# xuanvinh1997/llm-fp8

Measured on AMD Instinct MI355X. Metric: train tokens/sec + FP8 GEMM % of MFMA peak, Llama-3.2-3B seq512 b16, higher is better.
Workload: dtype fp8 (E4M3/E5M2 operands, fp32 accumulate, bf16 activations); 1 GPU; llama-3.2-3b (28 layers) full fine-tuning step, batch 16/GPU x seq 512, fp8_scenario=default (te_llama counterpart, lm_head FP8 under the outer recipe), random-init weights, synthetic tokens; route=fused, global_batch=16, seq_len=512, parallelism=single

## Files before the change

include/mi_fp8.h:

```cpp
#ifndef MI_FP8_H
#define MI_FP8_H

#include <stdint.h>

#ifdef __cplusplus
extern "C" {
#endif

#define MI_FMT_E4M3 0
#define MI_FMT_E5M2 1

#define MI_OK 0
#define MI_ERR_ARG (-1)
#define MI_ERR_SHAPE (-2)
#define MI_ERR_HIP (-3)

#define MI_OUT_BF16 0
#define MI_OUT_F32 1

#define MI_AMAX_ALGO_MAX 0
#define MI_AMAX_ALGO_MOST_RECENT 1

#define MI_ABI_VERSION 5
#define MI_ABI_REVISION 4
int mi_abi_version(void);
int mi_abi_revision(void);
const char* mi_last_error(void);
int mi_device_supported(void);

int mi_cast_amax(const void* x_bf16, void* y_fp8, void* yT_fp8, const float* scale, float* amax,
                 int64_t rows, int64_t cols, int64_t ld_y, int64_t ld_yT, int fmt, void* stream);
int mi_transpose_u8(const void* y, void* yT, int64_t rows, int64_t cols, int64_t ld_y, int64_t ld_yT, void* stream);
int mi_cast_amax_colsum(const void* x_bf16, void* y_fp8, void* yT_fp8, const float* scale, float* amax,
                        float* colsum_partial, int64_t rows, int64_t cols, int64_t ld_y, int64_t ld_yT, int fmt, void* stream);
int mi_colsum_finish(const float* partial, int64_t P, int64_t C, void* out, int out_dtype, void* stream);
int mi_colsum_finish_multi(const void* const* partials, const int64_t* P, const int64_t* C, void* const* outs,
                           const int* out_dtypes, int n, void* stream);

int mi_scale_update(float* amax_history, float* scale, float* scale_inv, const float* fp8_max,
// ... 119 lines not shown
                       const float* grad_scale, float lr, float beta1, float beta2, float eps, float weight_decay,
                       int64_t step, int sink_kind, void* stream);

int mi_adamw_sr_bf16_multi(const int64_t* table, int n_tensors, const int32_t* chunks, int n_chunks, int chunk_elems,
                           const float* grad_scale, float lr, float beta1, float beta2, float eps, float weight_decay,
                           int64_t step, int sink_kind, uint64_t seed, void* stream);

int mi_embedding_grad_add(void* grad_bf16, const void* dy_bf16, const int64_t* sorted_ids, const int64_t* perm, int64_t tokens,
                          int64_t hidden, int64_t vocab, float alpha, int64_t padding_idx, void* stream);
int mi_adamw_bf16(void* p_bf16, const void* g_bf16, void* exp_avg_bf16, void* exp_avg_sq_bf16, int64_t n,
                  const float* grad_scale, float lr, float beta1, float beta2, float eps, float weight_decay,
                  int64_t step, void* stream);

int mi_attn_fwd(const void* q, const void* k, const void* v, void* o, float* lse, int B, int S, int H, int G, int D,
                int64_t q_ts, int64_t k_ts, int64_t v_ts, int64_t o_ts, float scale, int causal, void* stream);
typedef struct mi_gemm_plan {
  int algo, family, build, sched, mx, tile_cfg, tiles_m, tiles_n, grid_x, grid_y, block, one_tile_per_wg, sk_units, bias_use;
} mi_gemm_plan;
#ifdef MI_DIAG
int mi_attn_fwd_diag(const void* q, const void* k, const void* v, void* o, float* lse, unsigned long long* dbg, int B, int S,
                     int H, int G, int D, int64_t q_ts, int64_t k_ts, int64_t v_ts, int64_t o_ts, float scale, void* stream);
int mi_gemm_plan_diag(int entry, int64_t M, int64_t N, int64_t K, int64_t lda, int64_t ldb, int64_t ldd, int fmt_a, int fmt_b,
                      int out_dtype, int has_bias, int algo, mi_gemm_plan* out);
#endif
int mi_attn_bwd(const void* q, const void* k, const void* v, const void* o, const void* dout, const float* lse,
                float* delta, void* dq, void* dk, void* dv, int B, int S, int H, int G, int D, int64_t q_ts,
                int64_t k_ts, int64_t v_ts, int64_t o_ts, int64_t do_ts, int64_t dq_ts, int64_t dk_ts, int64_t dv_ts,
                float scale, int causal, void* stream);

#ifdef __cplusplus
// ... 4 lines not shown
```

llm_fp8_amd/_lib.py:

```python
from __future__ import annotations

import ctypes
import os

_HERE = os.path.dirname(os.path.abspath(__file__))
LIB_PATH = os.environ.get("LLM_FP8_AMD_LIB") or os.path.join(_HERE, "libmi_fp8.so")
LAB_LIB_PATH = os.path.join(os.path.dirname(_HERE), "tools", "bin", "libmi_fp8_lab.so")

MI_FMT_E4M3 = 0
MI_FMT_E5M2 = 1
ABI_VERSION = 5
ABI_REVISION = 4

_c_i64 = ctypes.c_int64
_c_int = ctypes.c_int
_p = ctypes.c_void_p

class GemmProblem(ctypes.Structure):
    _fields_ = [("A", ctypes.c_void_p), ("B", ctypes.c_void_p), ("D", ctypes.c_void_p), ("sa_inv", ctypes.c_void_p),
                ("sb_inv", ctypes.c_void_p), ("M", ctypes.c_int64), ("N", ctypes.c_int64), ("K", ctypes.c_int64),
                ("lda", ctypes.c_int64), ("ldb", ctypes.c_int64), ("ldd", ctypes.c_int64)]


class GemmMxProblem(ctypes.Structure):
    _fields_ = [("A", ctypes.c_void_p), ("SA", ctypes.c_void_p), ("B", ctypes.c_void_p), ("SB", ctypes.c_void_p),
                ("D", ctypes.c_void_p), ("M", ctypes.c_int64), ("N", ctypes.c_int64), ("K", ctypes.c_int64)]

# ... 58 lines not shown
REVISION_SIGNATURES = {
    "mi_abi_revision": [],
    "mi_adamw_f32_multi": [_p, _c_int, _p, _c_int, _c_int, _p, ctypes.c_float, ctypes.c_float, ctypes.c_float, ctypes.c_float,
                           ctypes.c_float, _c_i64, _c_int, _p],
    "mi_amax_bf16": [_p, _p, _c_int, _c_i64, _c_i64, _p],
    "mi_amax_norm": [_p, _p, _p, _p, _c_int, _c_i64, _c_i64, _p],
    "mi_amax_swiglu": [_p, _p, _p, _c_int, _c_i64, _c_i64, _p],
    "mi_amax_dswiglu": [_p, _p, _p, _p, _c_int, _c_i64, _c_i64, _p],
    "mi_current_scale": [_p, _c_int, ctypes.c_float, ctypes.c_float, _c_int, _p, _p],
    "mi_blockfp8_quantize_ex": [_p, _p, _p, _p, _p, _p, _c_i64, _c_i64, _c_i64, _c_int, _c_int, ctypes.c_float, _p],
    "mi_blockfp8_norm_quantize": [_p, _p, _p, _p, _p, _p, _p, _c_i64, _c_i64, _c_int, _c_int, ctypes.c_float, _p],
    "mi_blockfp8_swiglu_quantize": [_p, _p, _p, _p, _p, _c_i64, _c_i64, _c_int, _c_int, ctypes.c_float, _p],
    "mi_blockfp8_dswiglu_quantize": [_p, _p, _p, _p, _p, _p, _p, _c_i64, _c_i64, _c_int, _c_int, ctypes.c_float, _p],
    "mi_adamw_sr_bf16_multi": [_p, _c_int, _p, _c_int, _c_int, _p, ctypes.c_float, ctypes.c_float, ctypes.c_float, ctypes.c_float,
                               ctypes.c_float, _c_i64, _c_int, ctypes.c_uint64, _p],
}
SIGNATURES.update(REVISION_SIGNATURES)
LAB_SIGNATURES = {
    "mi_attn_fwd_diag": [_p, _p, _p, _p, _p, _p, _c_int, _c_int, _c_int, _c_int, _c_int, _c_i64, _c_i64, _c_i64, _c_i64, ctypes.c_float, _p],
    "mi_gemm_plan_diag": [_c_int] + [_c_i64] * 6 + [_c_int] * 5 + [ctypes.POINTER(GemmPlan)],
}

_lib = None


def _bind(path: str, signatures) -> ctypes.CDLL:
    lib = ctypes.CDLL(path)
    for name, argtypes in signatures.items():
        if name in REVISION_SIGNATURES and not hasattr(lib, name):
            continue
# ... 54 lines not shown
```

llm_fp8_amd/csrc/mi_attn.hip:

```cpp
#include "mi_common.h"

namespace mi {

typedef __bf16 bf8 __attribute__((ext_vector_type(8)));
typedef short s4v __attribute__((ext_vector_type(4)));
typedef short s8v __attribute__((ext_vector_type(8)));
typedef float f16v __attribute__((ext_vector_type(16)));
typedef __attribute__((address_space(3))) s4v lds_s4v;

template <int D>
__device__ __forceinline__ int tile_off(int row, int ch) {
  if (D == 128) return 256 * row + 16 * (ch ^ (((row & 3) << 2) | ((row >> 2) & 3)));
  return 128 * row + 16 * (ch ^ (((row & 1) << 2) | ((row >> 1) & 3)));
}

__device__ __forceinline__ bf8 as_bf8(v4i v) { return __builtin_bit_cast(bf8, v); }

template <int D>
__device__ __forceinline__ bf8 row_frag(const char* tile, int r0, int t, int lane) {
  const int r = lane & 31, h = lane >> 5;
  return as_bf8(*reinterpret_cast<const v4i*>(tile + tile_off<D>(r0 + r, 2 * t + h)));
}

template <int D>
// ... 47 lines not shown
    __builtin_amdgcn_raw_ptr_buffer_load_lds(rs, MI_LDS_PTR(tile + (4 * i + w) * 1024), 16, voff[i], soff, 0, 0);
}
template <int D>
__device__ __forceinline__ void stage_dma_checked(rsrc_t rs, const int* voff, int adv, char* tile, int w) {
#pragma unroll
  for (int i = 0; i < D / 32; ++i)
    __builtin_amdgcn_raw_ptr_buffer_load_lds(rs, MI_LDS_PTR(tile + (4 * i + w) * 1024), 16, (int)((u32)voff[i] + (u32)adv), 0, 0, 0);
}
template <int D, bool TAIL>
__device__ __forceinline__ void stage_tile(rsrc_t rs, const int* voff, int adv, char* tile, int w) {
  if (TAIL) stage_dma_checked<D>(rs, voff, adv, tile, w);
  else stage_dma<D>(rs, voff, adv, tile, w);
}
__device__ __forceinline__ void dma_wait_all() { asm volatile("s_waitcnt vmcnt(0)" ::: "memory"); }

template <int D, bool CAUSAL, bool DIAG = false, bool TAIL = false>
__global__ __launch_bounds__(256, 2) void attn_fwd_kernel(const uint16_t* __restrict__ q, const uint16_t* __restrict__ k,
                                                          const uint16_t* __restrict__ v, uint16_t* __restrict__ o,
                                                          float* __restrict__ lse, int S, int H, int G, int64_t q_ts,
                                                          int64_t k_ts, int64_t v_ts, int64_t o_ts, float c,
                                                          unsigned long long* __restrict__ dbg = nullptr) {
  constexpr int TILE = ATT_KB * D * 2;
  constexpr int KT = D / 16, DB = D / 32;
  __shared__ __attribute__((aligned(16))) char lds[4 * TILE];
  const int tid = threadIdx.x, lane = tid & 63, w = tid >> 6, r = lane & 31, h = lane >> 5;
  const int qb = gridDim.x - 1 - blockIdx.x, head = blockIdx.y, b = blockIdx.z, g = head / (H / G);
  const int q_first = qb * ATT_QB + w * 32;
  const int qrow = q_first + r;
  int ntiles = CAUSAL ? (qb * ATT_QB + ATT_QB) / ATT_KB : S / ATT_KB;
  if (TAIL) {
    const int stiles = (S + ATT_KB - 1) / ATT_KB;
    ntiles = CAUSAL ? min(ntiles, stiles) : stiles;
  }
  const uint16_t* kbase = k + (int64_t)b * S * k_ts + (int64_t)g * D;
  const uint16_t* vbase = v + (int64_t)b * S * v_ts + (int64_t)g * D;

// ... 126 lines not shown
    MI_STAMP(2)
    dma_wait_all();
    MI_STAMP(3)
    __syncthreads();
    MI_STAMP(4)
  }
  if (DIAG && dbg != nullptr && lane == 0) {
    unsigned long long* dp = dbg + ((((int64_t)b * H + head) * gridDim.x + qb) * 4 + w) * 8;
    for (int i2 = 0; i2 < 5; ++i2) dp[i2] = tsum[i2];
    dp[5] = (unsigned long long)ntiles;
  }
#undef MI_STAMP

  l += __shfl_xor(l, 32);
  const float inv = 1.0f / l;
  if (h == 0 && (!TAIL || qrow < S)) lse[((int64_t)b * H + head) * S + qrow] = m * c + __builtin_amdgcn_logf(l);
  char* ot = lds + w * (32 * D * 2);
#pragma unroll
  for (int d = 0; d < DB; ++d)
#pragma unroll
    for (int i = 0; i < 4; ++i) {
      const int ch = 4 * d + i;
      uint2 pk;
      pk.x = pack_bf16x2(oacc[d][4 * i] * inv, oacc[d][4 * i + 1] * inv);
      pk.y = pack_bf16x2(oacc[d][4 * i + 2] * inv, oacc[d][4 * i + 3] * inv);
      *reinterpret_cast<uint2*>(ot + r * (D * 2) + 16 * (ch ^ (r & (D / 8 - 1))) + 8 * h) = pk;
    }
  __builtin_amdgcn_s_waitcnt(0xc07f);
  __builtin_amdgcn_wave_barrier();
  constexpr int CPR = D / 8;
#pragma unroll
  for (int it = 0; it < 32 * CPR / 64; ++it) {
    const int idx = it * 64 + lane, row = idx / CPR, ch = idx % CPR;
    const v4i val = *reinterpret_cast<const v4i*>(ot + row * (D * 2) + 16 * (ch ^ (row & (CPR - 1))));
    if (!TAIL || q_first + row < S) *reinterpret_cast<v4i*>(o + ((int64_t)b * S + q_first + row) * o_ts + (int64_t)head * D + ch * 8) = val;
  }
}


template <int D, bool TAIL = false>
__device__ __forceinline__ void store_rows_from_accT(const f16v (&acc)[D / 32], float mul, char* slice, uint16_t* out,
                                                     int64_t row_stride, int lane, int nrows = 32) {
  const int r = lane & 31, h = lane >> 5;
  constexpr int CPR = D / 8;
#pragma unroll
  for (int d = 0; d < D / 32; ++d)
#pragma unroll
    for (int i = 0; i < 4; ++i) {
      const int ch = 4 * d + i;
      uint2 pk;
// ... 304 lines not shown
#define MI_ATTN_FWD_T(DD, CC, TT)                                                                                      \
  hipLaunchKernelGGL((mi::attn_fwd_kernel<DD, CC, false, TT>), grid, block, 0, st, (const uint16_t*)q, (const uint16_t*)k, \
                     (const uint16_t*)v, (uint16_t*)o, lse, S, H, G, q_ts, k_ts, v_ts, o_ts, c, (unsigned long long*)nullptr)
#define MI_ATTN_FWD(DD, CC)                                                                                            \
  do {                                                                                                                 \
    if (tail) MI_ATTN_FWD_T(DD, CC, true); else MI_ATTN_FWD_T(DD, CC, false);                                          \
  } while (0)
  if (D == 128) {
    if (causal) MI_ATTN_FWD(128, true); else MI_ATTN_FWD(128, false);
  } else {
    if (causal) MI_ATTN_FWD(64, true); else MI_ATTN_FWD(64, false);
  }
#undef MI_ATTN_FWD_T
#undef MI_ATTN_FWD
  MI_CHECK_LAUNCH("mi_attn_fwd launch");
  return MI_OK;
}

#ifdef MI_DIAG
extern "C" int mi_attn_fwd_diag(const void* q, const void* k, const void* v, void* o, float* lse, unsigned long long* dbg, int B,
                                int S, int H, int G, int D, int64_t q_ts, int64_t k_ts, int64_t v_ts, int64_t o_ts, float scale,
                                void* stream) {
  MI_CHECK_ARG(q && k && v && o && lse && dbg, "mi_attn_fwd_diag: null pointer");
  MI_CHECK_ARG(D == 128 && S % 128 == 0 && H % G == 0, "mi_attn_fwd_diag: unsupported shape");
  dim3 grid(S / mi::ATT_QB, H, B), block(256);
  hipLaunchKernelGGL((mi::attn_fwd_kernel<128, true, true>), grid, block, 0, (hipStream_t)stream, (const uint16_t*)q,
                     (const uint16_t*)k, (const uint16_t*)v, (uint16_t*)o, lse, S, H, G, q_ts, k_ts, v_ts, o_ts,
                     scale * 1.4426950408889634f, dbg);
  MI_CHECK_LAUNCH("mi_attn_fwd_diag launch");
  return MI_OK;
// ... 46 lines not shown
```

llm_fp8_amd/pytorch/attention.py:

```python
from __future__ import annotations

import os
import weakref
from typing import Optional

import torch
import torch.nn.functional as F

from . import ops
from .module import DyHandoff, LayerNormLinear, Linear, handoff_readers

__all__ = ["RotaryPositionEmbedding", "apply_rotary_pos_emb", "DotProductAttention", "MultiheadAttention"]


class RotaryPositionEmbedding(torch.nn.Module):

    def __init__(self, dim: int, rotary_percent: float = 1.0, seq_len_interpolation_factor=None,
                 pretrained_max_position_embeddings=None, rotary_base: float = 10000.0):
        super().__init__()
        if rotary_percent < 1.0:
            dim = int(dim * rotary_percent)
        self.dim = dim
        self.seq_len_interpolation_factor = seq_len_interpolation_factor
        inv_freq = 1.0 / (rotary_base ** (torch.arange(0, dim, 2, dtype=torch.float32) / dim))
# ... 68 lines not shown
            if h.mx:
                fp8 = ops.mxfp8_rope_bwd_quantize(*args, h.fmt, rowwise=h.want_y, colwise=h.want_t)
            else:
                fp8 = ops.rope_qkv_backward_cast(*args, h.scale, h.amax, h.fmt, want_y=h.want_y, want_t=h.want_t)
            g = torch.empty((B, S, (n_q + 2 * n_kv) * d), dtype=torch.bfloat16, device=dq.device)
            h.put(fp8, g)
            return g, None, None, None, None, None, None
        g = ops.rope_qkv_backward(dq.reshape(T, n_q * d), dk.reshape(T, n_kv * d), dv.reshape(T, n_kv * d), cos, sin,
                                  n_q, n_kv, d, S)
        return g.view(B, S, -1), None, None, None, None, None, None


class _FlashAttnFn(torch.autograd.Function):

    @staticmethod
    def forward(ctx, q, k, v, scale, causal):
        o, lse = ops.attn_fwd(q, k, v, scale, causal)
        ctx.save_for_backward(q, k, v, o, lse)
        ctx.scale, ctx.causal = scale, causal
        return o

    @staticmethod
    def backward(ctx, do):
        q, k, v, o, lse = ctx.saved_tensors
        ok = (do.stride(3) == 1 and do.stride(2) == do.shape[3] and do.stride(0) == do.shape[1] * do.stride(1)
              and do.stride(1) % 8 == 0 and do.data_ptr() % 16 == 0)
        do = do if ok else do.clone(memory_format=torch.contiguous_format)
        dq, dk, dv = ops.attn_bwd(do, q, k, v, o, lse, ctx.scale, ctx.causal)
        return dq, dk, dv, None, None


def _flash_ok(q, k, v, causal: bool, dropout: float) -> bool:
    if not (q.is_cuda and q.dtype == k.dtype == v.dtype == torch.bfloat16 and dropout == 0.0 and causal):
        return False
    B, S, H, D = q.shape
    if D not in (64, 128) or S % 16 or S < 128 or H % k.shape[2]:
        return False
    return all(t.stride(3) == 1 and t.stride(2) == D and t.stride(0) == S * t.stride(1) and t.stride(1) % 8 == 0
               and S * t.stride(1) * 2 < 2 ** 31 and t.data_ptr() % 16 == 0 for t in (q, k, v))


class DotProductAttention(torch.nn.Module):

    def __init__(self, num_attention_heads: int, kv_channels: int, num_gqa_groups: Optional[int] = None,
                 attention_dropout: float = 0.0, attn_mask_type: str = "causal", qkv_format: str = "bshd", **_ignored):
        super().__init__()
        self.h, self.d = num_attention_heads, kv_channels
        self.g = num_gqa_groups or num_attention_heads
        self.p, self.attn_mask_type, self.qkv_format = attention_dropout, attn_mask_type, qkv_format

    def forward(self, q, k, v, attention_mask=None):
        if self.qkv_format == "sbhd":
            q, k, v = (t.transpose(0, 1) for t in (q, k, v))
        causal = self.attn_mask_type in ("causal", "padding_causal")
        if _flash_ok(q, k, v, causal, self.p if self.training else 0.0):
            o = _FlashAttnFn.apply(q, k, v, self.d ** -0.5, True)
            if self.qkv_format == "sbhd":
                o = o.transpose(0, 1)
            return o.reshape(*o.shape[:2], self.h * self.d)
        q, k, v = (t.transpose(1, 2) for t in (q, k, v))
        mask = None
        if not causal and attention_mask is not None:
            mask = ~attention_mask if attention_mask.dtype == torch.bool else attention_mask
        o = F.scaled_dot_product_attention(q, k, v, attn_mask=mask, dropout_p=self.p if self.training else 0.0,
                                           is_causal=causal, enable_gqa=(self.g != self.h))
        o = o.transpose(1, 2)
        if self.qkv_format == "sbhd":
            o = o.transpose(0, 1)
        return o.reshape(*o.shape[:2], self.h * self.d)


# ... 37 lines not shown
            if not self.input_layernorm:
                return self._attend(self.qkv(hidden_states), attention_mask, rotary_pos_emb), hidden_states
            handoff = DyHandoff() if (rotary_pos_emb is not None and hidden_states.is_cuda and torch.is_grad_enabled()
                                      and os.environ.get("LLM_FP8_AMD_NO_DY_HANDOFF") != "1") else None
            qkv, skip = self.layernorm_qkv(hidden_states, _with_skip=True, _rstd=_rstd, _dy_handoff=handoff)
            return self._attend(qkv, attention_mask, rotary_pos_emb, handoff), skip
        qkv = self.layernorm_qkv(hidden_states) if self.input_layernorm else self.qkv(hidden_states)
        return self._attend(qkv, attention_mask, rotary_pos_emb)

    def _attend(self, qkv: torch.Tensor, attention_mask, rotary_pos_emb, handoff=None) -> torch.Tensor:
        if (rotary_pos_emb is not None and not isinstance(rotary_pos_emb, (tuple, list)) and qkv.is_cuda
                and qkv.dtype == torch.bfloat16 and self.qkv_format == "bshd" and self.d % 16 == 0
                and rotary_pos_emb.shape[-1] == self.d):
            cos, sin = _cos_sin_tables(rotary_pos_emb, qkv.shape[1])
            q, k, v = _RoPESplitFn.apply(qkv, cos, sin, self.h, self.g, self.d, handoff)
            return self.proj(self.core_attention(q, k, v, attention_mask))
        if handoff is not None:
            handoff.withdraw()
        q, k, v = torch.split(qkv, self.split, dim=-1)
        a, b = qkv.shape[0], qkv.shape[1]
        q = q.reshape(a, b, self.h, self.d)
        k = k.reshape(a, b, self.g, self.d)
        v = v.reshape(a, b, self.g, self.d)
        if rotary_pos_emb is not None:
            fq, fk = rotary_pos_emb if isinstance(rotary_pos_emb, (tuple, list)) else (rotary_pos_emb, rotary_pos_emb)
            q = apply_rotary_pos_emb(q, fq, self.qkv_format)
            k = apply_rotary_pos_emb(k, fk, self.qkv_format)
        ctx = self.core_attention(q, k, v, attention_mask)
        return self.proj(ctx)
```

llm_fp8_amd/pytorch/module.py:

```python
from __future__ import annotations

import io
import os
from typing import List, Optional, Sequence, Tuple

import torch
import torch.nn.functional as F

from ..common.recipe import DelayedScaling, Float8BlockScaling, Float8CurrentScaling, Format, MXFP8BlockScaling, Recipe, fmt_codes
from . import ops
from .fp8 import FP8GlobalStateManager, ModuleMeta

__all__ = ["Linear", "LayerNormLinear", "LayerNormMLP", "LayerNorm", "RMSNorm"]


def _as_bf16_2d(t: torch.Tensor) -> torch.Tensor:
    t2 = t.reshape(-1, t.shape[-1])
    if t2.dtype != torch.bfloat16:
        t2 = t2.to(torch.bfloat16)
    return t2.contiguous()


class DyHandoff:
    __slots__ = ("scale", "amax", "fmt", "want_y", "want_t", "fp8", "ptr", "mx", "act_ref")
# ... 11 lines not shown

    def offered(self) -> bool:
        return (self.scale is not None or self.mx) and (self.want_y or self.want_t)

    def put(self, fp8: tuple, placeholder: torch.Tensor):
        self.fp8, self.ptr = fp8, placeholder.untyped_storage().data_ptr()

    def take(self, dy: torch.Tensor):
        if dy.untyped_storage().data_ptr() != self.ptr:
            raise RuntimeError("DyHandoff: the gradient reaching the Linear is not the producer's placeholder "
                               "(an op was inserted between the q|k|v projection and the rotary split)")
        fp8, self.fp8, self.ptr = self.fp8, None, None
        return fp8


def handoff_readers(t) -> bool:
    if torch.is_anomaly_enabled():
        return True
    if t is None:
        return False
    return bool(getattr(t, "retains_grad", False)) or bool(getattr(t, "_backward_hooks", None))


class _GemmSpec:
    __slots__ = ("recipe", "meta_fwd", "meta_bwd", "g", "fmt_fwd", "fmt_bwd", "trigger_bwd_update", "training", "eps",
                 "wcache", "first_mb", "with_skip", "rstd", "dy_handoff", "defer_bias", "q")

    def __init__(self, recipe, meta_fwd, meta_bwd, g, trigger_bwd_update, training, eps=1e-5, wcache=None, first_mb=None,
                 with_skip=False, rstd=None, dy_handoff=None, defer_bias=False):
        self.dy_handoff = dy_handoff
        self.defer_bias = defer_bias
        self.eps = eps
        self.rstd = rstd
        self.with_skip = with_skip
        self.wcache, self.first_mb = wcache, first_mb
        self.recipe, self.meta_fwd, self.meta_bwd, self.g = recipe, meta_fwd, meta_bwd, g
        self.fmt_fwd, self.fmt_bwd = fmt_codes(recipe.fp8_format)
        if recipe.mxfp8():
            self.q = _MXQ(self.fmt_fwd, self.fmt_bwd)
        elif recipe.current():
            self.q = _CurrentQ(recipe, self.fmt_fwd, self.fmt_bwd)
        elif recipe.block():
            self.q = _BlockQ(recipe, self.fmt_fwd, self.fmt_bwd)
        else:
            self.q = _DelayedQ(meta_fwd, meta_bwd, self.fmt_fwd, self.fmt_bwd)
# ... 101 lines not shown
    swiglu_adds_bias = True
    colsum_dtypes = None

    def __init__(self, mf, mb, fmt_f: int, fmt_b: int):
        self.mf, self.mb, self.fmt_f, self.fmt_b = mf, mb, fmt_f, fmt_b

    def _act(self, y, yT, s: int):
        return (y, self.mf.scale_inv(s)), (yT, self.mf.scale_inv_snapshot()[s:s + 1])

    def quantize(self, x2, g: int, want_t: bool, norm=None):
        mf, s = self.mf, 3 * g
        if norm is None:
            return self._act(*ops.cast_amax(x2, mf.scale(s), mf.amax(s), self.fmt_f, want_t=want_t), s)
        return self._act(*ops.norm_cast(x2, norm[0], norm[1], mf.scale(s), mf.amax(s), self.fmt_f, want_t=want_t), s)

    def swiglu(self, h, g: int, want_t: bool, bias):
        mf, s = self.mf, 3 * g
        return self._act(*ops.swiglu_cast(h, mf.scale(s), mf.amax(s), self.fmt_f, want_t=want_t, bias=bias), s)

    def _grad(self, y, yT, cs, s: int):
        si = self.mb.scale_inv(s)
        return (y, si), (yT, si), cs

    def quantize_grad(self, g2, g: int, want_y: bool, want_t: bool, colsum: bool = False):
        mb, s = self.mb, 2 * g
        out = ops.cast_amax(g2, mb.scale(s), mb.amax(s), self.fmt_b, want_y=want_y, want_t=want_t, want_colsum=colsum)
        return self._grad(out[0], out[1], out[2] if colsum else None, s)

    def dswiglu(self, h, dact, g: int, want_y: bool, want_t: bool, colsum: bool, bias):
        mb, s = self.mb, 2 * g
# ... 64 lines not shown

    def quantize_grad(self, g2, g: int, want_y: bool, want_t: bool, colsum: bool = False):
        q = ops.mxfp8_quantize(g2, self.fmt_b, rowwise=want_y, colwise=want_t, want_colsum=colsum)
        return q[:2], q[2:4], q[4] if colsum else None

    def dswiglu(self, h, dact, g: int, want_y: bool, want_t: bool, colsum: bool, bias):
        assert bias is None
        q = ops.mxfp8_dswiglu_quantize(h, dact, self.fmt_b, rowwise=want_y, colwise=want_t, want_colsum=colsum)
        return q[:2], q[2:4], q[4]

    def offer(self, handoff: DyHandoff, g: int, want_y: bool, want_t: bool) -> None:
        handoff.offer(None, None, self.fmt_b, want_y, want_t, mx=True)

    def taken(self, fp8, g: int):
        return fp8[:2], fp8[2:], None

    def operands(self, a, b):
        return a + b

    def gemm(self, a, b, bias):
        return ops.gemm_mxfp8(a[0], a[1], b[0], b[1], self.fmt_f, self.fmt_f, bias=bias)

    def unflat(self, flat):
        return flat[:2], flat[2:]

    def quantize_weights(self, weights, ns, N: int, K: int, dev, g: int, want_t: bool):
        fmt = self.fmt_f
        ws_ = [(w if w.dtype == torch.bfloat16 else w.to(torch.bfloat16)).contiguous() for w in weights]
        if len(ws_) == 1:
            return ops.mxfp8_quantize(ws_[0], fmt, rowwise=True, colwise=want_t)
# ... 135 lines not shown
        return (out[0], t3[2:3]), (out[1], t3[2:3]), out[2] if colsum else None

    def dswiglu(self, h, dact, g: int, want_y: bool, want_t: bool, colsum: bool, bias):
        part = ops.amax_partial(h.device, ops.amax_grid(h.shape[0], h.shape[1] // 2, 32))
        ops.amax_dswiglu(h, bias, dact, part)
        t3 = self._triple(part, self.fmt_b, self.recipe.fp8_quant_bwd_grad)
        y, yT, cs = ops.dswiglu_cast(h, dact, t3[1:2], None, self.fmt_b, want_y=want_y, want_t=want_t, want_colsum=colsum, bias=bias)
        return (y, t3[2:3]), (yT, t3[2:3]), cs

    def offer(self, handoff: DyHandoff, g: int, want_y: bool, want_t: bool) -> None:
        """Nothing: a DyHandoff producer needs the scale of grad_output before it has produced it.  RoPE backward and cross-entropy
        backward take their bf16 route and the Linear quantises the gradient it receives."""

    def taken(self, fp8, g: int):
        raise RuntimeError("Float8CurrentScaling offers no DyHandoff, so no producer can have put FP8 copies into one")

    operands = _DelayedQ.operands
    gemm = _DelayedQ.gemm
    unflat = _DelayedQ.unflat

    def quantize_weights(self, weights, ns, N: int, K: int, dev, g: int, want_t: bool):
        ws_ = [(w if w.dtype == torch.bfloat16 else w.to(torch.bfloat16)).contiguous() for w in weights]
        grids = [ops.amax_grid(n, K) for n in ns]
        part = ops.amax_partial(dev, sum(grids))
        o = 0
        for w, n in zip(ws_, grids):
            ops.amax_bf16(w, part[o:o + n])
            o += n
        t3 = self._triple(part, self.fmt_f, self.recipe.fp8_quant_fwd_weight)
        w8 = torch.empty((N, K), dtype=torch.uint8, device=dev)
# ... 108 lines not shown
    dx = gemm(*dgrad, fmt_b, fmt_f) if need_dgrad else None
    dw = gemm(*wgrad, fmt_b, fmt_f, out=dw_out) if need_wgrad else None
    return dx, dw


def _skip_2d(dskip: Optional[torch.Tensor], like: torch.Tensor) -> Optional[torch.Tensor]:
    if dskip is None:
        return None
    d = dskip.reshape(like.shape)
    return d if (d.dtype == torch.bfloat16 and d.is_contiguous()) else d.to(torch.bfloat16).contiguous()


def _quantize_input(ctx, spec: _GemmSpec, x2, ln_w, want_t: bool, need_dgrad: bool):
    ctx.norm = None
    if ln_w is None:
        return spec.q.quantize(x2, spec.g, want_t)
    gam = (ln_w if ln_w.dtype == torch.bfloat16 else ln_w.to(torch.bfloat16)).contiguous()
    rstd = spec.rstd if spec.rstd is not None else ops.rmsnorm_stats(x2, spec.eps)
    if need_dgrad:
        ctx.norm = (x2, rstd, gam, ln_w.dtype)
    return spec.q.quantize(x2, spec.g, want_t, (rstd, gam))


def _finish_dx(ctx, dx, dskip, colsums=None):
    dln = None
    if ctx.norm is not None and dx is not None:
        xin, rstd, gam, ln_dtype = ctx.norm
        ctx.norm = None
        dx, dln = ops.rmsnorm_bwd(dx, xin, rstd, gam, dres=_skip_2d(dskip, dx), dgamma_dtype=ln_dtype, finish=colsums is None)
        dskip = None
# ... 231 lines not shown
        torch.nn.init.normal_(w, mean=0.0, std=0.023)
    return torch.nn.Parameter(w)


class Linear(_FP8Module):

    def __init__(self, in_features: int, out_features: int, bias: bool = True, params_dtype=None, device="cuda",
                 init_method=None, **_ignored):
        super().__init__()
        self.in_features, self.out_features = in_features, out_features
        dt = params_dtype or torch.get_default_dtype()
        self.weight = _init_weight((out_features, in_features), dt, device, init_method)
        self.bias = torch.nn.Parameter(torch.zeros(out_features, dtype=dt, device=device)) if bias else None
        self.use_bias = bias

    def forward(self, inp: torch.Tensor, is_first_microbatch=None) -> torch.Tensor:
        st = self._prepare(inp.device)
        if st is None:
            if getattr(self, "_pending_norm", None) is not None:
                raise RuntimeError("Linear: a deferred RMSNorm is pending but FP8 is off for this forward")
            return F.linear(inp, _master(self.weight).to(inp.dtype), None if self.bias is None else self.bias.to(inp.dtype))
        handoff = DyHandoff() if (getattr(self, "offer_dy_handoff", False) and self.training and torch.is_grad_enabled()
                                  and self.bias is None) else None
        pn, self._pending_norm = getattr(self, "_pending_norm", None), None
        ln_w, eps, rstd = None, 1e-5, None
        if pn is not None:
            ln_w, eps, rs, ptr, shape = pn
            if inp.data_ptr() != ptr or tuple(inp.shape) != shape:
                raise RuntimeError("Linear: a deferred RMSNorm is pending for another tensor than the one this forward received")
            rstd = _usable_rstd(rs, inp, eps)
        y = _FP8LinearFn.apply(inp, self.bias, self._spec(st, is_first_microbatch, eps=eps, rstd=rstd, dy_handoff=handoff), ln_w,
                               self.weight)
        if handoff is not None and handoff.offered():
            y._mi_dy_handoff = handoff
        return y

    def extra_repr(self):
        return f"in_features={self.in_features}, out_features={self.out_features}, bias={self.use_bias}"


class LayerNormLinear(_FP8Module):

    def __init__(self, in_features: int, out_features: int, eps: float = 1e-5, bias: bool = True,
                 normalization: str = "LayerNorm", parameters_split=None, params_dtype=None, device="cuda",
                 zero_centered_gamma: bool = False, init_method=None, return_layernorm_output: bool = False, **_ignored):
        super().__init__()
        assert normalization in ("LayerNorm", "RMSNorm")
# ... 138 lines not shown
```

llm_fp8_amd/pytorch/ops.py:

```python
from __future__ import annotations

import ctypes
import os
from typing import Optional, Tuple

import torch

from .. import _lib
from .profiler import KernelTimer

E4M3, E5M2 = _lib.MI_FMT_E4M3, _lib.MI_FMT_E5M2
FP8_MAX = {E4M3: 448.0, E5M2: 57344.0}


_SK_WORKSPACE = {}


def ensure_gemm_workspace(device: torch.device) -> None:
    idx = device.index if device.index is not None else torch.cuda.current_device()
    if idx in _SK_WORKSPACE:
        return
    lib = _lib.load()
    with torch.cuda.device(idx):
        nbytes = int(lib.mi_gemm_workspace_bytes())
# ... 843 lines not shown
        _bshd_ok(o, D)
        assert o.shape == q.shape and lse.shape == (B, H, S) and lse.dtype == torch.float32 and lse.is_contiguous()
    args = (q.data_ptr(), k.data_ptr(), v.data_ptr(), o.data_ptr(), lse.data_ptr(), B, S, H, G, D, q.stride(1), k.stride(1),
            v.stride(1), o.stride(1), float(scale), int(causal), _stream())
    t = KernelTimer.active
    flops = 4.0 * B * H * S * S * D * (0.5 if causal else 1.0)
    if t is None:
        rc = _lib.load().mi_attn_fwd(*args)
    else:
        with t.span("attn_fwd", f"{B}x{S}x{H}x{D}", flops, 2.0 * (q.numel() * 2 + k.numel() * 2)):
            rc = _lib.load().mi_attn_fwd(*args)
    _lib.check(rc, "mi_attn_fwd")
    return o, lse


def attn_bwd(do: torch.Tensor, q: torch.Tensor, k: torch.Tensor, v: torch.Tensor, o: torch.Tensor, lse: torch.Tensor,
             scale: float, causal: bool = True, out=None):
    _dev(do, q, k, v, o, lse)
    B, S, H, D = q.shape
    G = k.shape[2]
    for t in (q, k, v, o, do):
        _bshd_ok(t, D)
    assert o.shape == do.shape == q.shape and lse.shape == (B, H, S) and lse.dtype == torch.float32 and lse.is_contiguous()
    if out is None:
        dq = torch.empty((B, S, H, D), dtype=torch.bfloat16, device=q.device)
        dk = torch.empty((B, S, G, D), dtype=torch.bfloat16, device=q.device)
        dv = torch.empty((B, S, G, D), dtype=torch.bfloat16, device=q.device)
    else:
        dq, dk, dv = out
        _dev(dq, dk, dv)
# ... 17 lines not shown
```

Baseline: 89910 tokens/s.

## Fuse FP8 cast and amax of attention output into flash-attention forward epilogue

Adds a CAST variant of the flash-attention forward kernel that, in its epilogue, converts the output tile to E4M3 with the output projection's delayed scale, publishes amax, and writes both row-major and LDS-transposed FP8 copies. A handoff object carries these copies to the o_proj Linear, which skips its own cast_amax kernel when the key matches. This removes a separate pass over the attention output and one kernel launch per layer. The cost is extra registers and LDS traffic in the attention epilogue, which could affect occupancy or scheduling, plus new Python plumbing.

```diff
diff --git a/include/mi_fp8.h b/include/mi_fp8.h
--- a/include/mi_fp8.h
+++ b/include/mi_fp8.h
@@ -22,7 +22,7 @@
 #define MI_AMAX_ALGO_MOST_RECENT 1
 
 #define MI_ABI_VERSION 5
-#define MI_ABI_REVISION 4
+#define MI_ABI_REVISION 5
 int mi_abi_version(void);
 int mi_abi_revision(void);
 const char* mi_last_error(void);
@@ -172,6 +172,9 @@
 
 int mi_attn_fwd(const void* q, const void* k, const void* v, void* o, float* lse, int B, int S, int H, int G, int D,
                 int64_t q_ts, int64_t k_ts, int64_t v_ts, int64_t o_ts, float scale, int causal, void* stream);
+int mi_attn_fwd_cast(const void* q, const void* k, const void* v, void* o, float* lse, void* y_fp8, void* yT_fp8,
+                     const float* scale_ptr, float* amax, int B, int S, int H, int G, int D, int64_t q_ts, int64_t k_ts,
+                     int64_t v_ts, int64_t ld_y, int64_t ld_yT, int fmt, float scale, int causal, void* stream);
 typedef struct mi_gemm_plan {
   int algo, family, build, sched, mx, tile_cfg, tiles_m, tiles_n, grid_x, grid_y, block, one_tile_per_wg, sk_units, bias_use;
 } mi_gemm_plan;
diff --git a/llm_fp8_amd/_lib.py b/llm_fp8_amd/_lib.py
--- a/llm_fp8_amd/_lib.py
+++ b/llm_fp8_amd/_lib.py
@@ -10,7 +10,7 @@
 MI_FMT_E4M3 = 0
 MI_FMT_E5M2 = 1
 ABI_VERSION = 5
-ABI_REVISION = 4
+ABI_REVISION = 5
 
 _c_i64 = ctypes.c_int64
 _c_int = ctypes.c_int
@@ -99,6 +99,7 @@
     "mi_blockfp8_dswiglu_quantize": [_p, _p, _p, _p, _p, _p, _p, _c_i64, _c_i64, _c_int, _c_int, ctypes.c_float, _p],
     "mi_adamw_sr_bf16_multi": [_p, _c_int, _p, _c_int, _c_int, _p, ctypes.c_float, ctypes.c_float, ctypes.c_float, ctypes.c_float,
                                ctypes.c_float, _c_i64, _c_int, ctypes.c_uint64, _p],
+    "mi_attn_fwd_cast": [_p] * 9 + [_c_int] * 5 + [_c_i64] * 5 + [_c_int, ctypes.c_float, _c_int, _p],
 }
 SIGNATURES.update(REVISION_SIGNATURES)
 LAB_SIGNATURES = {
diff --git a/llm_fp8_amd/csrc/mi_attn.hip b/llm_fp8_amd/csrc/mi_attn.hip
--- a/llm_fp8_amd/csrc/mi_attn.hip
+++ b/llm_fp8_amd/csrc/mi_attn.hip
@@ -85,12 +85,32 @@
 }
 __device__ __forceinline__ void dma_wait_all() { asm volatile("s_waitcnt vmcnt(0)" ::: "memory"); }
 
-template <int D, bool CAUSAL, bool DIAG = false, bool TAIL = false>
+struct FwdCast {
+  uint8_t* y;
+  uint8_t* yT;
+  const float* scale;
+  float* amax;
+  int64_t ld_y, ld_yT;
+};
+template <bool CAST>
+struct FwdLast { typedef unsigned long long* type; };
+template <>
+struct FwdLast<true> { typedef FwdCast type; };
+
+template <int D, bool CAUSAL, bool DIAG = false, bool TAIL = false, bool CAST = false>
 __global__ __launch_bounds__(256, 2) void attn_fwd_kernel(const uint16_t* __restrict__ q, const uint16_t* __restrict__ k,
                                                           const uint16_t* __restrict__ v, uint16_t* __restrict__ o,
                                                           float* __restrict__ lse, int S, int H, int G, int64_t q_ts,
                                                           int64_t k_ts, int64_t v_ts, int64_t o_ts, float c,
-                                                          unsigned long long* __restrict__ dbg = nullptr) {
+                                                          typename FwdLast<CAST>::type last = typename FwdLast<CAST>::type()) {
+  static_assert(!CAST || (D == 128 && CAUSAL && !DIAG && !TAIL), "the CAST form exists for head_dim 128, causal, whole blocks");
+  unsigned long long* __restrict__ dbg = nullptr;
+  if constexpr (!CAST) dbg = last;
+  float fp8_scale = 0.0f;
+  if constexpr (CAST) {
+    fp8_scale = *last.scale;
+    asm volatile("" : "+s"(fp8_scale));
+  }
   constexpr int TILE = ATT_KB * D * 2;
   constexpr int KT = D / 16, DB = D / 32;
   __shared__ __attribute__((aligned(16))) char lds[4 * TILE];
@@ -247,7 +267,7 @@
 
   l += __shfl_xor(l, 32);
   const float inv = 1.0f / l;
-  if (h == 0 && (!TAIL || qrow < S)) lse[((int64_t)b * H + head) * S + qrow] = m * c + __builtin_amdgcn_logf(l);
+  if (!CAST && h == 0 && (!TAIL || qrow < S)) lse[((int64_t)b * H + head) * S + qrow] = m * c + __builtin_amdgcn_logf(l);
   char* ot = lds + w * (32 * D * 2);
 #pragma unroll
   for (int d = 0; d < DB; ++d)
@@ -262,11 +282,71 @@
   __builtin_amdgcn_s_waitcnt(0xc07f);
   __builtin_amdgcn_wave_barrier();
   constexpr int CPR = D / 8;
+  [[maybe_unused]] u32 lo[8], hi[8];
+  [[maybe_unused]] const int rb = lane >> 4, cb = lane & 15;
+  if constexpr (CAST) {
+    v4i raw[8];
+#pragma unroll
+    for (int i = 0; i < 8; ++i) {
+      const int row = 8 * rb + i;
+      raw[i] = *reinterpret_cast<const v4i*>(ot + row * (D * 2) + 16 * (cb ^ (row & (CPR - 1))));
+    }
+    u32 screen = 0;
+#pragma unroll
+    for (int i = 0; i < 8; ++i)
+#pragma unroll
+      for (int j = 0; j < 4; ++j) screen = nan_screen(screen, (u32)raw[i][j]);
+    const bool has_nan = nan_seen(screen);
+    float amax = 0.0f;
+#pragma unroll
+    for (int i = 0; i < 8; ++i) {
+      float f[8];
+#pragma unroll
+      for (int j = 0; j < 4; ++j) {
+        const u32 wd = (u32)raw[i][j];
+        f[2 * j] = __uint_as_float(wd << 16);
+        f[2 * j + 1] = __uint_as_float(wd & 0xFFFF0000u);
+      }
+      if (__builtin_expect(has_nan, 0)) {
+#pragma unroll
+        for (int j = 0; j < 8; ++j) amax = fmaxf(amax, (f[j] != f[j]) ? 0.0f : fabsf(f[j]));
+      } else {
+#pragma unroll
+        for (int j = 0; j < 8; ++j) amax = fmaxf(amax, fabsf(f[j]));
+      }
+      lo[i] = cvt4_fp8<MI_FMT_E4M3>(f[0] * fp8_scale, f[1] * fp8_scale, f[2] * fp8_scale, f[3] * fp8_scale);
+      hi[i] = cvt4_fp8<MI_FMT_E4M3>(f[4] * fp8_scale, f[5] * fp8_scale, f[6] * fp8_scale, f[7] * fp8_scale);
+    }
+    publish_amax(amax, last.amax);
+    if (h == 0) lse[((int64_t)b * H + head) * S + qrow] = m * c + __builtin_amdgcn_logf(l);
+  }
 #pragma unroll
   for (int it = 0; it < 32 * CPR / 64; ++it) {
     const int idx = it * 64 + lane, row = idx / CPR, ch = idx % CPR;
     const v4i val = *reinterpret_cast<const v4i*>(ot + row * (D * 2) + 16 * (ch ^ (row & (CPR - 1))));
     if (!TAIL || q_first + row < S) *reinterpret_cast<v4i*>(o + ((int64_t)b * S + q_first + row) * o_ts + (int64_t)head * D + ch * 8) = val;
+  }
+  if constexpr (CAST) {
+    const FwdCast& fc = last;
+    const int64_t tok0 = (int64_t)b * S + (int64_t)qb * ATT_QB;
+    if (fc.y != nullptr)
+      store_rows8<MI_NT_Y>(fc.y + (tok0 + w * 32 + 8 * rb) * fc.ld_y + (int64_t)head * D + 8 * cb, fc.ld_y, lo, hi);
+    if (fc.yT != nullptr) {
+      char* ft = lds + 4 * (32 * D * 2);
+      const int br = 4 * w + rb;
+      char* wp = ft + 256 * br + 16 * (cb ^ br);
+#pragma unroll
+      for (int p = 0; p < 4; ++p) *reinterpret_cast<v4u*>(wp + 4096 * p) = v4u{lo[2 * p], hi[2 * p], lo[2 * p + 1], hi[2 * p + 1]};
+      __syncthreads();
+      const int br2 = lane & 15, bc2 = 4 * w + (lane >> 4);
+      const char* rp = ft + 256 * br2 + 16 * (bc2 ^ br2);
+#pragma unroll
+      for (int p = 0; p < 4; ++p) {
+        const v4u t4 = *reinterpret_cast<const v4u*>(rp + 4096 * p);
+        lo[2 * p] = t4[0]; hi[2 * p] = t4[1]; lo[2 * p + 1] = t4[2]; hi[2 * p + 1] = t4[3];
+      }
+      store_cols8<MI_NT_YT>(fc.yT + ((int64_t)head * D + 8 * bc2) * fc.ld_yT + tok0 + 8 * br2, fc.ld_yT, lo, hi);
+    }
   }
 }
 
@@ -601,6 +681,33 @@
 #undef MI_ATTN_FWD_T
 #undef MI_ATTN_FWD
   MI_CHECK_LAUNCH("mi_attn_fwd launch");
+  return MI_OK;
+}
+
+extern "C" int mi_attn_fwd_cast(const void* q, const void* k, const void* v, void* o, float* lse, void* y_fp8, void* yT_fp8,
+                                const float* scale_ptr, float* amax, int B, int S, int H, int G, int D, int64_t q_ts, int64_t k_ts,
+                                int64_t v_ts, int64_t ld_y, int64_t ld_yT, int fmt, float scale, int causal, void* stream) {
+  MI_CHECK_ARG(q && k && v && o && lse && scale_ptr, "mi_attn_fwd_cast: null pointer");
+  MI_CHECK_ARG(y_fp8 || yT_fp8, "mi_attn_fwd_cast: at least one of y, yT must be non-null");
+  MI_CHECK_ARG(B >= 1 && H >= 1 && G >= 1 && H % G == 0, "mi_attn_fwd_cast: bad B/H/G (%d, %d, %d)", B, H, G);
+  MI_CHECK_ARG(D == 128 && causal && S >= 128 && S % mi::ATT_QB == 0 && fmt == MI_FMT_E4M3,
+               "mi_attn_fwd_cast: only head_dim 128, causal, seq %% 128 == 0, E4M3 (got D %d, causal %d, S %d, fmt %d): use mi_attn_fwd + mi_cast_amax",
+               D, causal, S, fmt);
+  const int64_t M = (int64_t)B * S, C = (int64_t)H * D;
+  MI_CHECK_ARG(q_ts % 8 == 0 && k_ts % 8 == 0 && v_ts % 8 == 0, "mi_attn_fwd_cast: token strides must be multiples of 8");
+  MI_CHECK_ARG((int64_t)S * k_ts * 2 < (1LL << 31) && (int64_t)S * v_ts * 2 < (1LL << 31) && ((uintptr_t)k % 16) == 0 && ((uintptr_t)v % 16) == 0,
+               "mi_attn_fwd_cast: one batch of K / V must span < 2 GiB and be 16-byte aligned (32-bit buffer offsets of the LDS DMA)");
+  MI_CHECK_ARG(((uintptr_t)q % 16) == 0 && ((uintptr_t)o % 16) == 0, "mi_attn_fwd_cast: q and o must be 16-byte aligned (16-byte row accesses)");
+  MI_CHECK_ARG(!y_fp8 || (ld_y >= C && ld_y % 8 == 0), "mi_attn_fwd_cast: ld_y must be >= H * D and a multiple of 8");
+  MI_CHECK_ARG(!yT_fp8 || (ld_yT >= M && ld_yT % 8 == 0), "mi_attn_fwd_cast: ld_yT must be >= B * S and a multiple of 8");
+  MI_CHECK_ARG(((uintptr_t)y_fp8 % 8) == 0 && ((uintptr_t)yT_fp8 % 8) == 0, "mi_attn_fwd_cast: y / yT must be 8-byte aligned");
+  MI_CHECK_ARG(H <= 65535 && B <= 65535, "mi_attn_fwd_cast: grid too large");
+  const mi::FwdCast fc = {(uint8_t*)y_fp8, (uint8_t*)yT_fp8, scale_ptr, amax, ld_y, ld_yT};
+  dim3 grid(S / mi::ATT_QB, H, B), block(256);
+  hipLaunchKernelGGL((mi::attn_fwd_kernel<128, true, false, false, true>), grid, block, 0, (hipStream_t)stream, (const uint16_t*)q,
+                     (const uint16_t*)k, (const uint16_t*)v, (uint16_t*)o, lse, S, H, G, q_ts, k_ts, v_ts, C,
+                     scale * 1.4426950408889634f, fc);
+  MI_CHECK_LAUNCH("mi_attn_fwd_cast launch");
   return MI_OK;
 }
 
diff --git a/llm_fp8_amd/pytorch/attention.py b/llm_fp8_amd/pytorch/attention.py
--- a/llm_fp8_amd/pytorch/attention.py
+++ b/llm_fp8_amd/pytorch/attention.py
@@ -106,8 +106,12 @@
 class _FlashAttnFn(torch.autograd.Function):
 
     @staticmethod
-    def forward(ctx, q, k, v, scale, causal):
-        o, lse = ops.attn_fwd(q, k, v, scale, causal)
+    def forward(ctx, q, k, v, scale, causal, xh=None):
+        if xh is not None and xh.offered() and causal and ops.attn_fwd_cast_ok(q, xh.fmt):
+            o, lse, y, yT = ops.attn_fwd_cast(q, k, v, scale, xh.scale, xh.amax, xh.fmt, want_y=True, want_t=xh.want_t)
+            xh.put(y, yT, o)
+        else:
+            o, lse = ops.attn_fwd(q, k, v, scale, causal)
         ctx.save_for_backward(q, k, v, o, lse)
         ctx.scale, ctx.causal = scale, causal
         return o
@@ -119,7 +123,7 @@
               and do.stride(1) % 8 == 0 and do.data_ptr() % 16 == 0)
         do = do if ok else do.clone(memory_format=torch.contiguous_format)
         dq, dk, dv = ops.attn_bwd(do, q, k, v, o, lse, ctx.scale, ctx.causal)
-        return dq, dk, dv, None, None
+        return dq, dk, dv, None, None, None
 
 
 def _flash_ok(q, k, v, causal: bool, dropout: float) -> bool:
@@ -141,12 +145,13 @@
         self.g = num_gqa_groups or num_attention_heads
         self.p, self.attn_mask_type, self.qkv_format = attention_dropout, attn_mask_type, qkv_format
 
-    def forward(self, q, k, v, attention_mask=None):
+    def forward(self, q, k, v, attention_mask=None, _x_handoff=None):
         if self.qkv_format == "sbhd":
             q, k, v = (t.transpose(0, 1) for t in (q, k, v))
+            _x_handoff = None
         causal = self.attn_mask_type in ("causal", "padding_causal")
         if _flash_ok(q, k, v, causal, self.p if self.training else 0.0):
-            o = _FlashAttnFn.apply(q, k, v, self.d ** -0.5, True)
+            o = _FlashAttnFn.apply(q, k, v, self.d ** -0.5, True, _x_handoff)
             if self.qkv_format == "sbhd":
                 o = o.transpose(0, 1)
             return o.reshape(*o.shape[:2], self.h * self.d)
@@ -214,7 +219,10 @@
                 and rotary_pos_emb.shape[-1] == self.d):
             cos, sin = _cos_sin_tables(rotary_pos_emb, qkv.shape[1])
             q, k, v = _RoPESplitFn.apply(qkv, cos, sin, self.h, self.g, self.d, handoff)
-            return self.proj(self.core_attention(q, k, v, attention_mask))
+            xh = self.proj.offer_input(qkv.device) if isinstance(self.proj, Linear) else None
+            if xh is None:
+                return self.proj(self.core_attention(q, k, v, attention_mask))
+            return self.proj(self.core_attention(q, k, v, attention_mask, _x_handoff=xh), _x_handoff=xh)
         if handoff is not None:
             handoff.withdraw()
         q, k, v = torch.split(qkv, self.split, dim=-1)
diff --git a/llm_fp8_amd/pytorch/module.py b/llm_fp8_amd/pytorch/module.py
--- a/llm_fp8_amd/pytorch/module.py
+++ b/llm_fp8_amd/pytorch/module.py
@@ -49,6 +49,35 @@
         return fp8
 
 
+class XHandoff:
+    __slots__ = ("st", "scale", "amax", "fmt", "want_t", "fp8", "key")
+
+    def __init__(self, st):
+        self.st = st
+        self.scale = self.amax = self.fmt = self.fp8 = self.key = None
+        self.want_t = False
+
+    def offer(self, scale, amax, fmt, want_t: bool):
+        self.scale, self.amax, self.fmt, self.want_t = scale, amax, fmt, want_t
+
+    def offered(self) -> bool:
+        return self.scale is not None
+
+    @staticmethod
+    def _key(x: torch.Tensor):
+        return x.data_ptr(), x.numel(), x._version
+
+    def put(self, y, yT, x: torch.Tensor):
+        self.fp8, self.key = (y, yT), self._key(x)
+
+    def take(self, x2: torch.Tensor, want_t: bool):
+        fp8, key = self.fp8, self.key
+        self.fp8 = self.key = None
+        if fp8 is None or key != self._key(x2) or (want_t and fp8[1] is None):
+            return None
+        return fp8
+
+
 def handoff_readers(t) -> bool:
     if torch.is_anomaly_enabled():
         return True
@@ -59,11 +88,12 @@
 
 class _GemmSpec:
     __slots__ = ("recipe", "meta_fwd", "meta_bwd", "g", "fmt_fwd", "fmt_bwd", "trigger_bwd_update", "training", "eps",
-                 "wcache", "first_mb", "with_skip", "rstd", "dy_handoff", "defer_bias", "q")
+                 "wcache", "first_mb", "with_skip", "rstd", "dy_handoff", "x_handoff", "defer_bias", "q")
 
     def __init__(self, recipe, meta_fwd, meta_bwd, g, trigger_bwd_update, training, eps=1e-5, wcache=None, first_mb=None,
-                 with_skip=False, rstd=None, dy_handoff=None, defer_bias=False):
+                 with_skip=False, rstd=None, dy_handoff=None, defer_bias=False, x_handoff=None):
         self.dy_handoff = dy_handoff
+        self.x_handoff = x_handoff
         self.defer_bias = defer_bias
         self.eps = eps
         self.rstd = rstd
@@ -195,6 +225,13 @@
             return self._act(*ops.cast_amax(x2, mf.scale(s), mf.amax(s), self.fmt_f, want_t=want_t), s)
         return self._act(*ops.norm_cast(x2, norm[0], norm[1], mf.scale(s), mf.amax(s), self.fmt_f, want_t=want_t), s)
 
+    def offer_input(self, handoff: "XHandoff", g: int, want_t: bool) -> None:
+        if self.mf is not None:
+            handoff.offer(self.mf.scale(3 * g), self.mf.amax(3 * g), self.fmt_f, want_t)
+
+    def taken_input(self, fp8, g: int):
+        return self._act(fp8[0], fp8[1], 3 * g)
+
     def swiglu(self, h, g: int, want_t: bool, bias):
         mf, s = self.mf, 3 * g
         return self._act(*ops.swiglu_cast(h, mf.scale(s), mf.amax(s), self.fmt_f, want_t=want_t, bias=bias), s)
@@ -289,6 +326,9 @@
 
     def taken(self, fp8, g: int):
         return fp8[:2], fp8[2:], None
+
+    def offer_input(self, handoff: "XHandoff", g: int, want_t: bool) -> None:
+        """Nothing (here and under block scaling): the attention forward has no block-scaled form; the Linear quantises its input."""
 
     def operands(self, a, b):
         return a + b
@@ -454,6 +494,9 @@
 
     def taken(self, fp8, g: int):
         raise RuntimeError("Float8CurrentScaling offers no DyHandoff, so no producer can have put FP8 copies into one")
+
+    def offer_input(self, handoff: "XHandoff", g: int, want_t: bool) -> None:
+        """Nothing: the scale of the input comes from its own amax, which the producer has not got before it has produced it."""
 
     operands = _DelayedQ.operands
     gemm = _DelayedQ.gemm
@@ -592,6 +635,9 @@
 def _quantize_input(ctx, spec: _GemmSpec, x2, ln_w, want_t: bool, need_dgrad: bool):
     ctx.norm = None
     if ln_w is None:
+        fp8 = spec.x_handoff.take(x2, want_t) if spec.x_handoff is not None else None
+        if fp8 is not None:
+            return spec.q.taken_input(fp8, spec.g)
         return spec.q.quantize(x2, spec.g, want_t)
     gam = (ln_w if ln_w.dtype == torch.bfloat16 else ln_w.to(torch.bfloat16)).contiguous()
     rstd = spec.rstd if spec.rstd is not None else ops.rmsnorm_stats(x2, spec.eps)
@@ -853,8 +899,18 @@
         self.bias = torch.nn.Parameter(torch.zeros(out_features, dtype=dt, device=device)) if bias else None
         self.use_bias = bias
 
-    def forward(self, inp: torch.Tensor, is_first_microbatch=None) -> torch.Tensor:
-        st = self._prepare(inp.device)
+    def offer_input(self, device) -> Optional[XHandoff]:
+        if os.environ.get("LLM_FP8_AMD_NO_ATTN_OUT_HANDOFF") == "1" or getattr(self, "_pending_norm", None) is not None:
+            return None
+        st = self._prepare(device)
+        if st is None:
+            return None
+        xh = XHandoff(st)
+        self._spec(st, None).q.offer_input(xh, 0, self.weight.requires_grad and torch.is_grad_enabled())
+        return xh
+
+    def forward(self, inp: torch.Tensor, is_first_microbatch=None, _x_handoff: Optional[XHandoff] = None) -> torch.Tensor:
+        st = self._prepare(inp.device) if _x_handoff is None else _x_handoff.st
         if st is None:
             if getattr(self, "_pending_norm", None) is not None:
                 raise RuntimeError("Linear: a deferred RMSNorm is pending but FP8 is off for this forward")
@@ -868,8 +924,8 @@
             if inp.data_ptr() != ptr or tuple(inp.shape) != shape:
                 raise RuntimeError("Linear: a deferred RMSNorm is pending for another tensor than the one this forward received")
             rstd = _usable_rstd(rs, inp, eps)
-        y = _FP8LinearFn.apply(inp, self.bias, self._spec(st, is_first_microbatch, eps=eps, rstd=rstd, dy_handoff=handoff), ln_w,
-                               self.weight)
+        y = _FP8LinearFn.apply(inp, self.bias, self._spec(st, is_first_microbatch, eps=eps, rstd=rstd, dy_handoff=handoff,
+                                                          x_handoff=_x_handoff), ln_w, self.weight)
         if handoff is not None and handoff.offered():
             y._mi_dy_handoff = handoff
         return y
diff --git a/llm_fp8_amd/pytorch/ops.py b/llm_fp8_amd/pytorch/ops.py
--- a/llm_fp8_amd/pytorch/ops.py
+++ b/llm_fp8_amd/pytorch/ops.py
@@ -881,6 +881,38 @@
     return o, lse
 
 
+def attn_fwd_cast_ok(q: torch.Tensor, fmt: int) -> bool:
+    B, S, H, D = q.shape
+    return D == 128 and S % 128 == 0 and (B * S) % 8 == 0 and fmt == E4M3
+
+
+def attn_fwd_cast(q: torch.Tensor, k: torch.Tensor, v: torch.Tensor, scale: float, fp8_scale: torch.Tensor,
+                  amax: Optional[torch.Tensor], fmt: int, want_y: bool = True, want_t: bool = True):
+    _dev(q, k, v, fp8_scale, amax)
+    B, S, H, D = q.shape
+    G = k.shape[2]
+    for t in (q, k, v):
+        _bshd_ok(t, D)
+    assert attn_fwd_cast_ok(q, fmt) and (want_y or want_t)
+    assert fp8_scale.dtype == torch.float32 and (amax is None or amax.dtype == torch.float32)
+    M, C = B * S, H * D
+    o = torch.empty((B, S, H, D), dtype=torch.bfloat16, device=q.device)
+    lse = torch.empty((B, H, S), dtype=torch.float32, device=q.device)
+    y = torch.empty((M, C), dtype=torch.uint8, device=q.device) if want_y else None
+    yT = torch.empty((C, M), dtype=torch.uint8, device=q.device) if want_t else None
+    fn = _lib.require("mi_attn_fwd_cast", "the attention forward that emits the output projection's FP8 input")
+    args = (q.data_ptr(), k.data_ptr(), v.data_ptr(), o.data_ptr(), lse.data_ptr(), _ptr(y), _ptr(yT), fp8_scale.data_ptr(),
+            _ptr(amax), B, S, H, G, D, q.stride(1), k.stride(1), v.stride(1), C, M, fmt, float(scale), 1, _stream())
+    t = KernelTimer.active
+    if t is None:
+        rc = fn(*args)
+    else:
+        with t.span("attn_fwd", f"{B}x{S}x{H}x{D}", 2.0 * B * H * S * S * D, 2.0 * (q.numel() * 2 + k.numel() * 2)):
+            rc = fn(*args)
+    _lib.check(rc, "mi_attn_fwd_cast")
+    return o, lse, y, yT
+
+
 def attn_bwd(do: torch.Tensor, q: torch.Tensor, k: torch.Tensor, v: torch.Tensor, o: torch.Tensor, lse: torch.Tensor,
              scale: float, causal: bool = True, out=None):
     _dev(do, q, k, v, o, lse)
```

Result: no change. 90250 tokens/s, median of 5 (+0.4%).
